# showlab/EgoVLP

Hardware: NVIDIA H100
Metric: clips/sec, 16-frame TimeSformer-B + DistilBERT + EgoNCE training step (higher is better)
Workload: dtype bf16

## Files before the change

### egovlp_b200/csrc/common.cuh

```cuda
#pragma once
#include <cuda.h>
#include <cuda_bf16.h>
#include <cuda_runtime.h>
#include <stdint.h>
#include <stdio.h>

#define EGOVLP_OK 0
#define EGOVLP_ERR_ARG (-1)
#define EGOVLP_ERR_CUDA (-2)
#define EGOVLP_ERR_UNSUPPORTED (-3)

namespace egovlp {

typedef __nv_bfloat16 bf16;

void set_last_error(const char* fmt, ...);

#define EGOVLP_CHECK_ARG(cond, ...)                                   \
  do {                                                                \
    if (!(cond)) {                                                    \
      ::egovlp::set_last_error(__VA_ARGS__);                          \
      return EGOVLP_ERR_ARG;                                          \
    }                                                                 \
  } while (0)
// ... 126 lines not shown
      "cp.async.bulk.tensor.2d.shared::cluster.global.mbarrier::complete_tx::bytes [%0], [%1, {%3, %4}], [%2];"
      ::"r"(dst), "l"(reinterpret_cast<uint64_t>(m)), "r"(bar), "r"(c0), "r"(c1)
      : "memory");
}
__device__ __forceinline__ void tma_load_3d(uint32_t dst, const CUtensorMap* m, uint32_t bar, int c0, int c1, int c2) {
  asm volatile(
      "cp.async.bulk.tensor.3d.shared::cluster.global.mbarrier::complete_tx::bytes [%0], [%1, {%3, %4, %5}], [%2];"
      ::"r"(dst), "l"(reinterpret_cast<uint64_t>(m)), "r"(bar), "r"(c0), "r"(c1), "r"(c2)
      : "memory");
}
__device__ __forceinline__ void tma_load_4d(uint32_t dst, const CUtensorMap* m, uint32_t bar, int c0, int c1, int c2,
                                            int c3) {
  asm volatile(
      "cp.async.bulk.tensor.4d.shared::cluster.global.mbarrier::complete_tx::bytes [%0], [%1, {%3, %4, %5, %6}], [%2];"
      ::"r"(dst), "l"(reinterpret_cast<uint64_t>(m)), "r"(bar), "r"(c0), "r"(c1), "r"(c2), "r"(c3)
      : "memory");
}
__device__ __forceinline__ void tma_load_5d(uint32_t dst, const CUtensorMap* m, uint32_t bar, int c0, int c1, int c2,
                                            int c3, int c4) {
  asm volatile(
      "cp.async.bulk.tensor.5d.shared::cluster.global.mbarrier::complete_tx::bytes [%0], [%1, {%3, %4, %5, %6, %7}], [%2];"
      ::"r"(dst), "l"(reinterpret_cast<uint64_t>(m)), "r"(bar), "r"(c0), "r"(c1), "r"(c2), "r"(c3), "r"(c4)
      : "memory");
}
__device__ __forceinline__ void tma_load_2d_multicast(uint32_t dst, const CUtensorMap* m, uint32_t bar, int c0, int c1,
                                                      uint16_t mask) {
  asm volatile(
      "cp.async.bulk.tensor.2d.shared::cluster.global.mbarrier::complete_tx::bytes.multicast::cluster"
      " [%0], [%1, {%3, %4}], [%2], %5;"
      ::"r"(dst), "l"(reinterpret_cast<uint64_t>(m)), "r"(bar), "r"(c0), "r"(c1), "h"(mask)
      : "memory");
}
__device__ __forceinline__ void fence_proxy_async_smem() {
  asm volatile("fence.proxy.async.shared::cta;" ::: "memory");
}
__device__ __forceinline__ void bulk_load_1d(uint32_t dst, const void* src, uint32_t bytes, uint32_t bar) {
  asm volatile("cp.async.bulk.shared::cluster.global.mbarrier::complete_tx::bytes [%0], [%1], %2, [%3];"
               ::"r"(dst), "l"(reinterpret_cast<uint64_t>(src)), "r"(bytes), "r"(bar)
               : "memory");
}
__device__ __forceinline__ void tma_store_2d(const CUtensorMap* m, uint32_t src, int c0, int c1) {
  asm volatile("cp.async.bulk.tensor.2d.global.shared::cta.bulk_group [%0, {%2, %3}], [%1];"
               ::"l"(reinterpret_cast<uint64_t>(m)), "r"(src), "r"(c0), "r"(c1)
               : "memory");
}
__device__ __forceinline__ void bulk_commit() { asm volatile("cp.async.bulk.commit_group;" ::: "memory"); }
template <int N>
__device__ __forceinline__ void bulk_wait_read() { asm volatile("cp.async.bulk.wait_group.read %0;" ::"n"(N) : "memory"); }
template <int N>
__device__ __forceinline__ void bulk_wait() { asm volatile("cp.async.bulk.wait_group %0;" ::"n"(N) : "memory"); }
__device__ __forceinline__ void named_bar_sync(int id, int count) {
  asm volatile("bar.sync %0, %1;" ::"r"(id), "r"(count) : "memory");
}

__device__ __forceinline__ uint32_t cluster_ctarank() {
  uint32_t r;
  asm volatile("mov.u32 %0, %%cluster_ctarank;" : "=r"(r));
  return r;
}
__device__ __forceinline__ void cluster_sync_all() {
  asm volatile("barrier.cluster.arrive.release.aligned;\n\tbarrier.cluster.wait.acquire.aligned;" ::: "memory");
}
__device__ __forceinline__ uint32_t mapa_shared(uint32_t addr, uint32_t cta_rank) {
  uint32_t r;
  asm volatile("mapa.shared::cluster.u32 %0, %1, %2;" : "=r"(r) : "r"(addr), "r"(cta_rank));
  return r;
}
__device__ __forceinline__ void mbar_arrive_cluster(uint32_t cluster_addr) {
  asm volatile("mbarrier.arrive.release.cluster.shared::cluster.b64 _, [%0];" ::"r"(cluster_addr) : "memory");
}

__device__ __forceinline__ void wgmma_fence() { asm volatile("wgmma.fence.sync.aligned;" ::: "memory"); }
__device__ __forceinline__ void wgmma_commit() { asm volatile("wgmma.commit_group.sync.aligned;" ::: "memory"); }
template <int N>
__device__ __forceinline__ void wgmma_wait() { asm volatile("wgmma.wait_group.sync.aligned %0;" ::"n"(N) : "memory"); }
template <int R>
__device__ __forceinline__ void wgmma_fence_regs(float (&d)[R]) {
#pragma unroll
  for (int i = 0; i < R; ++i) asm volatile("" : "+f"(d[i])::"memory");
}

__device__ __forceinline__ uint64_t make_smem_desc_sw128(uint32_t saddr, uint32_t lbo_bytes, uint32_t sbo_bytes) {
  uint64_t d = 0;
  d |= uint64_t((saddr >> 4) & 0x3FFF);
  d |= uint64_t((lbo_bytes >> 4) & 0x3FFF) << 16;
  d |= uint64_t((sbo_bytes >> 4) & 0x3FFF) << 32;
  d |= uint64_t(1) << 62;
  return d;
}

int make_tmap_2d_bf16(CUtensorMap* out, const void* base, uint64_t rows, uint64_t cols, uint64_t ld, uint32_t box_rows,
                      uint32_t box_cols);
int make_tmap_2d_f32(CUtensorMap* out, const void* base, uint64_t rows, uint64_t cols, uint64_t ld, uint32_t box_rows,
                     uint32_t box_cols);
int make_tmap_nd_bf16(CUtensorMap* out, const void* base, int rank, const uint64_t* dims, const uint64_t* strides,
                      const uint32_t* box, bool swizzle128);

}
```

### egovlp_b200/csrc/gemm_wgmma.cu

```cuda
#include <stdlib.h>

#include "common.cuh"
#include "egovlp_b200.h"

namespace egovlp {

namespace {

constexpr int BLOCK_M = 128;
constexpr int BLOCK_K = 64;
constexpr int WG_K = 16;
constexpr int A_STAGE_BYTES = BLOCK_M * BLOCK_K * 2;
constexpr int MN_ATOM_BYTES = BLOCK_K * 128;
constexpr int NUM_THREADS = 384;

struct EpiParams {
  const float* bias;
  const float* residual;
  const bf16* aux;
  void* out;
  bf16* out2;
  long long ldr, ldaux, ldo, ldo2;
  int out_mode;
  int act;
  float alpha;
  float col_scale;
  int col_scale_ncols;
  int res_row_mod;
  float* colsum;
  float* colsum_a;
};

constexpr int EPI_ROWS = 64;
constexpr int EPI_SUB_BYTES = EPI_ROWS * 128;
constexpr int EPI_BUFS = 2;
constexpr int EPI_BIAS_BYTES = 256 * 4;
constexpr int EPI_SMEM_BYTES = 2 * EPI_BUFS * EPI_SUB_BYTES + EPI_BIAS_BYTES;

template <int BLOCK_N>
struct Cfg {
  static constexpr int B_STAGE_BYTES = BLOCK_N * BLOCK_K * 2;
  static constexpr int STAGES = BLOCK_N == 256 ? 4 : 6;
  static constexpr int ACC = BLOCK_N / 2;
  static constexpr int RING_BYTES = STAGES * (A_STAGE_BYTES + B_STAGE_BYTES);
  static constexpr int SMEM_BYTES = RING_BYTES + 1024  + 256 ;
  static constexpr int SMEM_BYTES_STAGED = SMEM_BYTES + EPI_SMEM_BYTES;
  static_assert(SMEM_BYTES_STAGED <= 232448, "shared memory per block");
};

__device__ __forceinline__ void red_add_v4(float* p, float a, float b, float c, float d) {
  asm volatile("red.global.add.v4.f32 [%0], {%1, %2, %3, %4};" ::"l"(p), "f"(a), "f"(b), "f"(c), "f"(d) : "memory");
}
__device__ __forceinline__ void red_add_v2(float* p, float a, float b) {
  asm volatile("red.global.add.v2.f32 [%0], {%1, %2};" ::"l"(p), "f"(a), "f"(b) : "memory");
}

template <int TA, int TB>
__device__ __forceinline__ void wgmma_m64n256k16(float (&d)[128], uint64_t adesc, uint64_t bdesc, int scale_d) {
  asm volatile(
      "{\n\t.reg .pred p;\n\t"
      "setp.ne.b32 p, %130, 0;\n\t"
      "wgmma.mma_async.sync.aligned.m64n256k16.f32.bf16.bf16 "
      "{%0,%1,%2,%3,%4,%5,%6,%7,%8,%9,%10,%11,%12,%13,%14,%15,%16,%17,%18,%19,%20,%21,%22,%23,%24,%25,%26,%27,%28,%29,%30,%31,"
      "%32,%33,%34,%35,%36,%37,%38,%39,%40,%41,%42,%43,%44,%45,%46,%47,%48,%49,%50,%51,%52,%53,%54,%55,%56,%57,%58,%59,%60,%61,%62,%63,"
      "%64,%65,%66,%67,%68,%69,%70,%71,%72,%73,%74,%75,%76,%77,%78,%79,%80,%81,%82,%83,%84,%85,%86,%87,%88,%89,%90,%91,%92,%93,%94,%95,"
      "%96,%97,%98,%99,%100,%101,%102,%103,%104,%105,%106,%107,%108,%109,%110,%111,%112,%113,%114,%115,%116,%117,%118,%119,%120,%121,%122,%123,%124,%125,%126,%127}, "
      "%128, %129, p, 1, 1, %131, %132;\n\t}"
      : "+f"(d[0]), "+f"(d[1]), "+f"(d[2]), "+f"(d[3]), "+f"(d[4]), "+f"(d[5]), "+f"(d[6]), "+f"(d[7]),
        "+f"(d[8]), "+f"(d[9]), "+f"(d[10]), "+f"(d[11]), "+f"(d[12]), "+f"(d[13]), "+f"(d[14]), "+f"(d[15]),
        "+f"(d[16]), "+f"(d[17]), "+f"(d[18]), "+f"(d[19]), "+f"(d[20]), "+f"(d[21]), "+f"(d[22]), "+f"(d[23]),
        "+f"(d[24]), "+f"(d[25]), "+f"(d[26]), "+f"(d[27]), "+f"(d[28]), "+f"(d[29]), "+f"(d[30]), "+f"(d[31]),
        "+f"(d[32]), "+f"(d[33]), "+f"(d[34]), "+f"(d[35]), "+f"(d[36]), "+f"(d[37]), "+f"(d[38]), "+f"(d[39]),
        "+f"(d[40]), "+f"(d[41]), "+f"(d[42]), "+f"(d[43]), "+f"(d[44]), "+f"(d[45]), "+f"(d[46]), "+f"(d[47]),
        "+f"(d[48]), "+f"(d[49]), "+f"(d[50]), "+f"(d[51]), "+f"(d[52]), "+f"(d[53]), "+f"(d[54]), "+f"(d[55]),
        "+f"(d[56]), "+f"(d[57]), "+f"(d[58]), "+f"(d[59]), "+f"(d[60]), "+f"(d[61]), "+f"(d[62]), "+f"(d[63]),
        "+f"(d[64]), "+f"(d[65]), "+f"(d[66]), "+f"(d[67]), "+f"(d[68]), "+f"(d[69]), "+f"(d[70]), "+f"(d[71]),
        "+f"(d[72]), "+f"(d[73]), "+f"(d[74]), "+f"(d[75]), "+f"(d[76]), "+f"(d[77]), "+f"(d[78]), "+f"(d[79]),
        "+f"(d[80]), "+f"(d[81]), "+f"(d[82]), "+f"(d[83]), "+f"(d[84]), "+f"(d[85]), "+f"(d[86]), "+f"(d[87]),
        "+f"(d[88]), "+f"(d[89]), "+f"(d[90]), "+f"(d[91]), "+f"(d[92]), "+f"(d[93]), "+f"(d[94]), "+f"(d[95]),
        "+f"(d[96]), "+f"(d[97]), "+f"(d[98]), "+f"(d[99]), "+f"(d[100]), "+f"(d[101]), "+f"(d[102]), "+f"(d[103]),
        "+f"(d[104]), "+f"(d[105]), "+f"(d[106]), "+f"(d[107]), "+f"(d[108]), "+f"(d[109]), "+f"(d[110]), "+f"(d[111]),
        "+f"(d[112]), "+f"(d[113]), "+f"(d[114]), "+f"(d[115]), "+f"(d[116]), "+f"(d[117]), "+f"(d[118]), "+f"(d[119]),
        "+f"(d[120]), "+f"(d[121]), "+f"(d[122]), "+f"(d[123]), "+f"(d[124]), "+f"(d[125]), "+f"(d[126]), "+f"(d[127])
      : "l"(adesc), "l"(bdesc), "r"(scale_d), "n"(TA), "n"(TB));
}
template <int TA, int TB>
__device__ __forceinline__ void wgmma_m64n128k16(float (&d)[64], uint64_t adesc, uint64_t bdesc, int scale_d) {
  asm volatile(
      "{\n\t.reg .pred p;\n\t"
// ... 35 lines not shown
  u = mul2(x, gc.k);
  float u0, u1, a0, a1, t0, t1, e0, e1, r0, r1;
  up2(u, u0, u1);
  asm("rcp.approx.ftz.f32 %0, %1;" : "=f"(t0) : "f"(fmaf(fabsf(u0), GELU_PT, 1.f)));
  asm("rcp.approx.ftz.f32 %0, %1;" : "=f"(t1) : "f"(fmaf(fabsf(u1), GELU_PT, 1.f)));
  up2(fma2(mul2(x, gc.nk), u, gc.l2c), a0, a1);
  asm("ex2.approx.ftz.f32 %0, %1;" : "=f"(e0) : "f"(a0));
  asm("ex2.approx.ftz.f32 %0, %1;" : "=f"(e1) : "f"(a1));
  const f32x2 t = pk2(t0, t1);
  e = pk2(e0, e1);
  f32x2 p = fma2(t, gc.b5, gc.b4);
  p = fma2(p, t, gc.b3);
  p = fma2(p, t, gc.b2);
  p = fma2(p, t, gc.b1);
  up2(fma2(mul2(p, t), e, gc.half), r0, r1);
  return add2(pk2(copysignf(r0, x0), copysignf(r1, x1)), gc.half);
}
__device__ __forceinline__ void gelu2(const GeluConsts& gc, float& x0, float& x1) {
  const f32x2 x = pk2(x0, x1);
  f32x2 u, e;
  up2(mul2(x, gelu_phi2(gc, x0, x1, x, u, e)), x0, x1);
}
__device__ __forceinline__ void gelu_and_grad2(const GeluConsts& gc, float x0, float x1, uint32_t& g_bf, uint32_t& d_bf) {
  const f32x2 x = pk2(x0, x1);
  f32x2 u, e;
  const f32x2 phi = gelu_phi2(gc, x0, x1, x, u, e);
  float g0, g1, d0, d1;
  up2(mul2(x, phi), g0, g1);
  up2(fma2(u, e, phi), d0, d1);
  g_bf = pack_bf16x2(g0, g1);
  d_bf = pack_bf16x2(d0, d1);
}
__device__ __forceinline__ float gelu_grad_fast(float x) {
  float t;
  asm("rcp.approx.ftz.f32 %0, %1;" : "=f"(t) : "f"(fmaf(fabsf(x), 0.3275911f * 0.70710678118654752f, 1.f)));
  const float e = exp2f(x * x * -0.72134752044448170f);
  float p = fmaf(t, 0.5f * 1.061405429f, 0.5f * -1.453152027f);
  p = fmaf(p, t, 0.5f * 1.421413741f);
  p = fmaf(p, t, 0.5f * -0.284496736f);
  p = fmaf(p, t, 0.5f * 0.254829592f);
  const float phi_cdf = 0.5f + copysignf(fmaf(-(p * t), e, 0.5f), x);
  return fmaf(x * 0.3989422804014327f, e, phi_cdf);
}

enum EpiMode {
  EPI_GENERIC = 0,
  EPI_BF16 = 1,
  EPI_ACT3 = 2,
  EPI_MUL_AUX = 3,
  EPI_RES_F32 = 4,
  EPI_ACT1 = 5,
};

template <int BLOCK_N, bool A_MN, bool B_MN, bool TWO, int MODE>
__global__ void __launch_bounds__(NUM_THREADS, 1)
gemm_bf16_wgmma_kernel(const __grid_constant__ CUtensorMap tmA, const __grid_constant__ CUtensorMap tmB,
                       const __grid_constant__ CUtensorMap tmOut, const __grid_constant__ CUtensorMap tmOut2,
                       const __grid_constant__ CUtensorMap tmIn, int M, int N, int K, int num_m_blocks,
                       int num_n_blocks, int kb_per_split, int num_splits, EpiParams ep) {
  static_assert(!(TWO && A_MN && B_MN), "the wgrad form (column sums of A) runs on single CTAs");
  using C = Cfg<BLOCK_N>;
  constexpr int TILE_M = TWO ? 2 * BLOCK_M : BLOCK_M;
  const uint32_t rank = TWO ? cluster_ctarank() : 0u;
  const int worker = TWO ? (int)(blockIdx.x >> 1) : (int)blockIdx.x;
  const int num_workers = TWO ? (int)(gridDim.x >> 1) : (int)gridDim.x;
  constexpr int STAGES = C::STAGES;
  constexpr bool STAGED = MODE != EPI_GENERIC;
  constexpr bool OUT_F32 = MODE == EPI_RES_F32;
  constexpr bool HAS_IN = MODE == EPI_RES_F32 || MODE == EPI_MUL_AUX;
  constexpr bool TWO_OUT = MODE == EPI_ACT3;
  constexpr int SUB_COLS = OUT_F32 ? 32 : 64;
  constexpr int NSUB = BLOCK_N / SUB_COLS;
  extern __shared__ uint8_t smem_raw[];
  const uint32_t smem_base = (smem_u32(smem_raw) + 1023u) & ~1023u;
  const uint32_t sA = smem_base;
  const uint32_t sB = smem_base + STAGES * A_STAGE_BYTES;
  const uint32_t sEpi = sB + STAGES * C::B_STAGE_BYTES;
  const uint32_t sBias = sEpi + 2 * EPI_BUFS * EPI_SUB_BYTES;
  const uint32_t bars = STAGED ? sBias + EPI_BIAS_BYTES : sEpi;
  const uint32_t full_bar = bars;
  const uint32_t empty_bar = bars + 8 * STAGES;
  const uint32_t epi_full = bars + 16 * STAGES;
  const uint32_t epi_empty = epi_full + 8 * 2 * EPI_BUFS;
  const uint32_t bias_full = epi_empty + 8 * 2 * EPI_BUFS;
  const uint32_t bias_empty = bias_full + 8;

  const int warp = threadIdx.x >> 5;
  const int lane = threadIdx.x & 31;
  const int num_tiles = num_m_blocks * num_n_blocks;
  const int num_units = num_tiles * num_splits;
  const int num_kb = (K + BLOCK_K - 1) / BLOCK_K;
  const bool sum_a = A_MN && B_MN && ep.colsum_a != nullptr;

  if (threadIdx.x == 0) {
    tma_prefetch_desc(&tmA);
    tma_prefetch_desc(&tmB);
    for (int s = 0; s < STAGES; ++s) {
      mbar_init(full_bar + 8 * s, 1);
      mbar_init(empty_bar + 8 * s, (TWO || sum_a) ? 4 : 2);
    }
    if (STAGED) {
      tma_prefetch_desc(&tmOut);
      if (TWO_OUT) tma_prefetch_desc(&tmOut2);
      if (HAS_IN) tma_prefetch_desc(&tmIn);
      for (int i = 0; i < 2 * EPI_BUFS; ++i) {
        mbar_init(epi_full + 8 * i, 1);
        mbar_init(epi_empty + 8 * i, 1);
      }
      mbar_init(bias_full, 1);
      mbar_init(bias_empty, 2);
    }
    fence_mbar_init();
  }
  if (STAGED && !ep.bias && threadIdx.x < BLOCK_N)
    asm volatile("st.shared.f32 [%0], %1;" ::"r"(sBias + 4 * threadIdx.x), "f"(0.f) : "memory");
  if (TWO) cluster_sync_all();
  else __syncthreads();

  if (warp < 4) {
    asm volatile("setmaxnreg.dec.sync.aligned.u32 40;");
    if (warp == 0) {
      if (lane == 0) {
        int stage = 0;
        uint32_t phase = 0;
        for (int unit = worker; unit < num_units; unit += num_workers) {
          const int split = unit / num_tiles, tile = unit - split * num_tiles;
          const int m_blk = tile / num_n_blocks, n_blk = tile - m_blk * num_n_blocks;
          const int kb0 = split * kb_per_split, kb1 = min(num_kb, kb0 + kb_per_split);
          const int m_row = m_blk * TILE_M + (int)rank * BLOCK_M, n_row = n_blk * BLOCK_N;
          for (int kb = kb0; kb < kb1; ++kb) {
            mbar_wait_nocall(empty_bar + 8 * stage, phase ^ 1);
            const uint32_t fb = full_bar + 8 * stage;
            mbar_expect_tx(fb, A_STAGE_BYTES + C::B_STAGE_BYTES);
            const uint32_t a_dst = sA + stage * A_STAGE_BYTES, b_dst = sB + stage * C::B_STAGE_BYTES;
            if (!A_MN) {
              tma_load_2d(a_dst, &tmA, fb, kb * BLOCK_K, m_row);
            } else {
#pragma unroll
              for (int i = 0; i < BLOCK_M / 64; ++i)
                tma_load_2d(a_dst + i * MN_ATOM_BYTES, &tmA, fb, m_row + i * 64, kb * BLOCK_K);
            }
            if (TWO) {
              if (!B_MN) {
                tma_load_2d_multicast(b_dst + rank * (BLOCK_N / 2) * 128, &tmB, fb, kb * BLOCK_K,
                                      n_row + (int)rank * (BLOCK_N / 2), 3);
              } else {
#pragma unroll
                for (int i = 0; i < BLOCK_N / 128; ++i) {
                  const int slab = (int)rank * (BLOCK_N / 128) + i;
                  tma_load_2d_multicast(b_dst + slab * MN_ATOM_BYTES, &tmB, fb, n_row + slab * 64, kb * BLOCK_K, 3);
                }
              }
            } else if (!B_MN) {
              tma_load_2d(b_dst, &tmB, fb, kb * BLOCK_K, n_row);
            } else {
#pragma unroll
              for (int i = 0; i < BLOCK_N / 64; ++i)
                tma_load_2d(b_dst + i * MN_ATOM_BYTES, &tmB, fb, n_row + i * 64, kb * BLOCK_K);
            }
            if (++stage == STAGES) { stage = 0; phase ^= 1; }
          }
        }
      }
    } else if ((warp == 2 || warp == 3) && sum_a) {
      const int slab = warp - 2, chunk = lane & 7, rsub = lane >> 3;
      int stage = 0;
      uint32_t phase = 0;
      for (int unit = worker; unit < num_units; unit += num_workers) {
        const int split = unit / num_tiles, tile = unit - split * num_tiles;
        const int m_blk = tile / num_n_blocks, n_blk = tile - m_blk * num_n_blocks;
        const int kb0 = split * kb_per_split, kb1 = min(num_kb, kb0 + kb_per_split);
        float acc[8];
#pragma unroll
        for (int j = 0; j < 8; ++j) acc[j] = 0.f;
        for (int kb = kb0; kb < kb1; ++kb) {
          mbar_wait_nocall(full_bar + 8 * stage, phase);
          if (kb % num_n_blocks == n_blk) {
            const uint32_t slab_base = sA + stage * A_STAGE_BYTES + slab * MN_ATOM_BYTES;
#pragma unroll 4
            for (int i = 0; i < 16; ++i) {
              const int r = rsub + 4 * i;
              uint32_t v0, v1, v2, v3;
              asm volatile("ld.shared.v4.u32 {%0, %1, %2, %3}, [%4];"
                           : "=r"(v0), "=r"(v1), "=r"(v2), "=r"(v3)
                           : "r"(slab_base + r * 128 + ((chunk ^ (r & 7)) << 4)));
              acc[0] += __uint_as_float(v0 << 16); acc[1] += __uint_as_float(v0 & 0xffff0000u);
              acc[2] += __uint_as_float(v1 << 16); acc[3] += __uint_as_float(v1 & 0xffff0000u);
              acc[4] += __uint_as_float(v2 << 16); acc[5] += __uint_as_float(v2 & 0xffff0000u);
              acc[6] += __uint_as_float(v3 << 16); acc[7] += __uint_as_float(v3 & 0xffff0000u);
            }
          }
          __syncwarp();
          if (lane == 0) mbar_arrive(empty_bar + 8 * stage);
          if (++stage == STAGES) { stage = 0; phase ^= 1; }
        }
#pragma unroll
        for (int j = 0; j < 8; ++j) {
          acc[j] += __shfl_xor_sync(0xffffffffu, acc[j], 8);
          acc[j] += __shfl_xor_sync(0xffffffffu, acc[j], 16);
        }
        const int col = m_blk * BLOCK_M + slab * 64 + chunk * 8;
        if (lane < 8 && col < M) {
          red_add_v4(ep.colsum_a + col, acc[0], acc[1], acc[2], acc[3]);
          red_add_v4(ep.colsum_a + col + 4, acc[4], acc[5], acc[6], acc[7]);
        }
      }
    } else if (STAGED && warp == 1) {
      if (lane == 0) {
        uint32_t it = 0, tc = 0;
        for (int unit = worker; unit < num_units; unit += num_workers, ++tc) {
          const int m_blk = unit / num_n_blocks, n_blk = unit - m_blk * num_n_blocks;
          const int m_row = m_blk * TILE_M + (int)rank * BLOCK_M, n0 = n_blk * BLOCK_N;
          mbar_wait_nocall(bias_empty, (tc & 1) ^ 1);
          if (ep.bias) {
            const uint32_t bytes = 4u * (uint32_t)min(BLOCK_N, N - n0);
            mbar_expect_tx(bias_full, bytes);
            bulk_load_1d(sBias, ep.bias + n0, bytes, bias_full);
          } else {
            mbar_arrive(bias_full);
          }
          if (HAS_IN) {
            for (int s = 0; s < NSUB; ++s, ++it) {
              const uint32_t b = it % EPI_BUFS, ph = (it / EPI_BUFS) & 1;
#pragma unroll
              for (int w = 0; w < 2; ++w) {
                const uint32_t slot = w * EPI_BUFS + b;
                mbar_wait_nocall(epi_empty + 8 * slot, ph ^ 1);
                mbar_expect_tx(epi_full + 8 * slot, EPI_SUB_BYTES);
                tma_load_2d(sEpi + slot * EPI_SUB_BYTES, &tmIn, epi_full + 8 * slot, n0 + s * SUB_COLS,
                            m_row + w * EPI_ROWS);
              }
            }
          }
        }
      }
    }
  } else {
    asm volatile("setmaxnreg.inc.sync.aligned.u32 232;");
    const int mw = (threadIdx.x >> 7) - 1;
    const bool leader = (threadIdx.x & 127) == 0;
    auto release = [&](int st) {
      const uint32_t bar = empty_bar + 8 * st;
      if (TWO) { mbar_arrive_cluster(mapa_shared(bar, 0)); mbar_arrive_cluster(mapa_shared(bar, 1)); }
      else mbar_arrive(bar);
    };
    const int wq = warp & 3;
    const GeluConsts gc;

    float acc[C::ACC];
    int stage = 0;
    uint32_t phase = 0;
    uint32_t it = 0, tc = 0;
    for (int unit = worker; unit < num_units; unit += num_workers, ++tc) {
      const int split = unit / num_tiles, tile = unit - split * num_tiles;
      const int m_blk = tile / num_n_blocks, n_blk = tile - m_blk * num_n_blocks;
      const int kb0 = split * kb_per_split, kb1 = min(num_kb, kb0 + kb_per_split);
      int prev_stage = -1;
      for (int kb = kb0; kb < kb1; ++kb) {
        mbar_wait_nocall(full_bar + 8 * stage, phase);
        const uint32_t a_src = sA + stage * A_STAGE_BYTES + mw * (64 * 128), b_src = sB + stage * C::B_STAGE_BYTES;
        wgmma_fence_regs(acc);
        wgmma_fence();
#pragma unroll
        for (int k = 0; k < BLOCK_K / WG_K; ++k) {
          const uint64_t adesc = A_MN ? make_smem_desc_sw128(a_src + k * (WG_K * 128), MN_ATOM_BYTES, 1024)
                                      : make_smem_desc_sw128(a_src + k * (WG_K * 2), 16, 1024);
          const uint64_t bdesc = B_MN ? make_smem_desc_sw128(b_src + k * (WG_K * 128), MN_ATOM_BYTES, 1024)
                                      : make_smem_desc_sw128(b_src + k * (WG_K * 2), 16, 1024);
          wgmma_tile<BLOCK_N, A_MN ? 1 : 0, B_MN ? 1 : 0>(acc, adesc, bdesc, (kb > kb0 || k > 0) ? 1 : 0);
        }
        wgmma_commit();
        wgmma_fence_regs(acc);
        wgmma_wait<1>();
        wgmma_fence_regs(acc);
        if (prev_stage >= 0 && leader) release(prev_stage);
        prev_stage = stage;
        if (++stage == STAGES) { stage = 0; phase ^= 1; }
      }
      wgmma_wait<0>();
      wgmma_fence_regs(acc);
      if (leader) release(prev_stage);

      if constexpr (STAGED) {
        const int m_row = m_blk * TILE_M + (int)rank * BLOCK_M + mw * EPI_ROWS, n0 = n_blk * BLOCK_N;
        const int c2 = 2 * (lane & 3);
        mbar_wait_nocall(bias_full, tc & 1);
#pragma unroll
        for (int s = 0; s < NSUB; ++s, ++it) {
          const uint32_t b = it % EPI_BUFS, ph = (it / EPI_BUFS) & 1;
          if (TWO_OUT) named_bar_sync(1 + mw, 128);
          const uint32_t buf = sEpi + (mw * EPI_BUFS + (TWO_OUT ? 0u : b)) * EPI_SUB_BYTES;
          if (HAS_IN) mbar_wait_nocall(epi_full + 8 * (mw * EPI_BUFS + b), ph);
#pragma unroll
          for (int jj = 0; jj < SUB_COLS / 8; ++jj) {
            const int j = s * (SUB_COLS / 8) + jj;
            float2 bq;
            asm volatile("ld.shared.v2.f32 {%0, %1}, [%2];" : "=f"(bq.x), "=f"(bq.y) : "r"(sBias + 4 * (8 * j + c2)));
#pragma unroll
            for (int h = 0; h < 2; ++h) {
              const int r = wq * 16 + (lane >> 2) + 8 * h;
              const uint32_t off = OUT_F32 ? r * 128 + (((2 * jj + ((lane & 3) >> 1)) ^ (r & 7)) << 4) + 8 * (lane & 1)
                                           : r * 128 + ((jj ^ (r & 7)) << 4) + 4 * (lane & 3);
              float v0 = __fmaf_rn(acc[4 * j + 2 * h], ep.alpha, bq.x);
              float v1 = __fmaf_rn(acc[4 * j + 2 * h + 1], ep.alpha, bq.y);
              if (MODE == EPI_BF16 && n0 + 8 * j + c2 < ep.col_scale_ncols) {
                v0 = __fmul_rn(v0, ep.col_scale); v1 = __fmul_rn(v1, ep.col_scale);
              }
              if (MODE == EPI_ACT3) {
                uint32_t g, d;
                gelu_and_grad2(gc, v0, v1, g, d);
                asm volatile("st.shared.u32 [%0], %1;" ::"r"(buf + off), "r"(g) : "memory");
                asm volatile("st.shared.u32 [%0], %1;" ::"r"(buf + EPI_SUB_BYTES + off), "r"(d) : "memory");
              } else if (MODE == EPI_RES_F32) {
                float r0, r1;
                asm volatile("ld.shared.v2.f32 {%0, %1}, [%2];" : "=f"(r0), "=f"(r1) : "r"(buf + off) : "memory");
                v0 += r0; v1 += r1;
                asm volatile("st.shared.v2.f32 [%0], {%1, %2};" ::"r"(buf + off), "f"(v0), "f"(v1) : "memory");
              } else {
                if (MODE == EPI_ACT1) gelu2(gc, v0, v1);
                if (MODE == EPI_MUL_AUX) {
                  uint32_t a;
                  asm volatile("ld.shared.u32 %0, [%1];" : "=r"(a) : "r"(buf + off) : "memory");
                  const float2 af = unpack_bf16x2(a);
                  v0 *= af.x; v1 *= af.y;
                }
                asm volatile("st.shared.u32 [%0], %1;" ::"r"(buf + off), "r"(pack_bf16x2(v0, v1)) : "memory");
              }
            }
          }
          fence_proxy_async_smem();
          named_bar_sync(1 + mw, 128);
          if (leader) {
            tma_store_2d(&tmOut, buf, n0 + s * SUB_COLS, m_row);
            if (TWO_OUT) tma_store_2d(&tmOut2, buf + EPI_SUB_BYTES, n0 + s * SUB_COLS, m_row);
            bulk_commit();
            bulk_wait_read<0>();
            if (HAS_IN) mbar_arrive(epi_empty + 8 * (mw * EPI_BUFS + b));
          }
        }
        if (leader) mbar_arrive(bias_empty);
      } else {
      const int row_lo = m_blk * TILE_M + (int)rank * BLOCK_M + mw * 64 + wq * 16 + (lane >> 2);
      const int col_base = n_blk * BLOCK_N + 2 * (lane & 3);
#pragma unroll
      for (int j = 0; j < BLOCK_N / 8; ++j) {
        const int col = col_base + 8 * j;
        if (n_blk * BLOCK_N + 8 * j >= N) break;
        float2 bq = make_float2(0.f, 0.f);
        if (ep.bias) bq = __ldg(reinterpret_cast<const float2*>(ep.bias + col));
        float cs0 = 0.f, cs1 = 0.f;
#pragma unroll
        for (int h = 0; h < 2; ++h) {
          const int row = row_lo + 8 * h;
          const bool rv = row < M;
          float v0 = __fmaf_rn(acc[4 * j + 2 * h], ep.alpha, bq.x);
          float v1 = __fmaf_rn(acc[4 * j + 2 * h + 1], ep.alpha, bq.y);
          if (col < ep.col_scale_ncols) { v0 = __fmul_rn(v0, ep.col_scale); v1 = __fmul_rn(v1, ep.col_scale); }
          if (ep.act == 3) {
            uint32_t g, d;
            gelu_and_grad2(gc, v0, v1, g, d);
            if (rv) {
              *reinterpret_cast<uint32_t*>(reinterpret_cast<bf16*>(ep.out) + (long long)row * ep.ldo + col) = g;
              if (ep.out2) *reinterpret_cast<uint32_t*>(ep.out2 + (long long)row * ep.ldo2 + col) = d;
            }
            continue;
          }
          if (ep.out2 && rv)
            *reinterpret_cast<uint32_t*>(ep.out2 + (long long)row * ep.ldo2 + col) = pack_bf16x2(v0, v1);
          if (ep.act == 1) gelu2(gc, v0, v1);
          const int grow = rv ? row : M - 1;
          if (ep.act == 2 || ep.act == 4) {
            const float2 a = unpack_bf16x2(__ldg(reinterpret_cast<const unsigned int*>(ep.aux + (long long)grow * ep.ldaux + col)));
            if (ep.act == 2) { v0 *= gelu_grad_fast(a.x); v1 *= gelu_grad_fast(a.y); }
            else { v0 *= a.x; v1 *= a.y; }
          }
          if (ep.residual) {
            const int rrow = ep.res_row_mod ? grow % ep.res_row_mod : grow;
            const float2 r = __ldg(reinterpret_cast<const float2*>(ep.residual + (long long)rrow * ep.ldr + col));
            v0 += r.x; v1 += r.y;
          }
          if (!rv) continue;
          cs0 += v0; cs1 += v1;
          if (ep.out_mode == 0) {
            *reinterpret_cast<uint32_t*>(reinterpret_cast<bf16*>(ep.out) + (long long)row * ep.ldo + col) = pack_bf16x2(v0, v1);
          } else if (ep.out_mode == 1) {
            *reinterpret_cast<float2*>(reinterpret_cast<float*>(ep.out) + (long long)row * ep.ldo + col) = make_float2(v0, v1);
          } else {
            red_add_v2(reinterpret_cast<float*>(ep.out) + (long long)row * ep.ldo + col, v0, v1);
          }
        }
        if (ep.colsum) {
#pragma unroll
          for (int o = 4; o < 32; o <<= 1) {
            cs0 += __shfl_xor_sync(0xffffffffu, cs0, o);
            cs1 += __shfl_xor_sync(0xffffffffu, cs1, o);
          }
          if (lane < 4) red_add_v2(ep.colsum + col, cs0, cs1);
        }
      }
      }
    }
    if (STAGED && leader) bulk_wait<0>();
  }
  if (TWO) cluster_sync_all();
}

template <int BLOCK_N, bool A_MN, bool B_MN, bool TWO, int MODE = EPI_GENERIC>
int launch(const void* A, long long lda, const void* B, long long ldb, int M, int N, int K, int splits,
           const EpiParams& ep, cudaStream_t stream) {
  using C = Cfg<BLOCK_N>;
  CUtensorMap tmA, tmB;
  int rc;
  if (!A_MN) rc = make_tmap_2d_bf16(&tmA, A, M, K, lda, BLOCK_M, BLOCK_K);
  else       rc = make_tmap_2d_bf16(&tmA, A, K, M, lda, BLOCK_K, 64);
  if (rc) return rc;
  if (!B_MN) rc = make_tmap_2d_bf16(&tmB, B, N, K, ldb, TWO ? BLOCK_N / 2 : BLOCK_N, BLOCK_K);
  else       rc = make_tmap_2d_bf16(&tmB, B, K, N, ldb, BLOCK_K, 64);
  if (rc) return rc;
  constexpr bool STAGED = MODE != EPI_GENERIC;
  CUtensorMap tmOut = {}, tmOut2 = {}, tmIn = {};
  if (MODE == EPI_RES_F32) {
    rc = make_tmap_2d_f32(&tmOut, ep.out, M, N, ep.ldo, EPI_ROWS, 32);
    if (!rc) rc = make_tmap_2d_f32(&tmIn, ep.residual, M, N, ep.ldr, EPI_ROWS, 32);
  } else if (STAGED) {
    rc = make_tmap_2d_bf16(&tmOut, ep.out, M, N, ep.ldo, EPI_ROWS, 64);
    if (!rc && MODE == EPI_ACT3) rc = make_tmap_2d_bf16(&tmOut2, ep.out2, M, N, ep.ldo2, EPI_ROWS, 64);
    if (!rc && MODE == EPI_MUL_AUX) rc = make_tmap_2d_bf16(&tmIn, ep.aux, M, N, ep.ldaux, EPI_ROWS, 64);
  }
  if (rc) return rc;
  constexpr int SMEM_BYTES = STAGED ? C::SMEM_BYTES_STAGED : C::SMEM_BYTES;
  constexpr int TILE_M = TWO ? 2 * BLOCK_M : BLOCK_M;
  const int num_m_blocks = (M + TILE_M - 1) / TILE_M, num_n_blocks = (N + BLOCK_N - 1) / BLOCK_N;
  const int num_kb = (K + BLOCK_K - 1) / BLOCK_K;
  splits = max(1, min(splits, num_kb));
  const int kb_per_split = (num_kb + splits - 1) / splits;
  splits = (num_kb + kb_per_split - 1) / kb_per_split;
  const int units = num_m_blocks * num_n_blocks * splits;
  auto kern = gemm_bf16_wgmma_kernel<BLOCK_N, A_MN, B_MN, TWO, MODE>;
  static bool attr_set = false;
  if (!attr_set) {
    EGOVLP_CHECK_CUDA(cudaFuncSetAttribute(kern, cudaFuncAttributeMaxDynamicSharedMemorySize, SMEM_BYTES));
    attr_set = true;
  }
  cudaLaunchConfig_t cfg = {};
  cudaLaunchAttribute attr[1];
  cfg.blockDim = dim3(NUM_THREADS);
  cfg.dynamicSmemBytes = SMEM_BYTES;
  cfg.stream = stream;
  if (TWO) {
    attr[0].id = cudaLaunchAttributeClusterDimension;
    attr[0].val.clusterDim.x = 2;
    attr[0].val.clusterDim.y = 1;
    attr[0].val.clusterDim.z = 1;
    cfg.attrs = attr;
    cfg.numAttrs = 1;
  }
  static int resident = 0;
  if (!resident) {
    if (TWO) {
      cfg.gridDim = dim3(num_sms() & ~1);
      EGOVLP_CHECK_CUDA(cudaOccupancyMaxActiveClusters(&resident, kern, &cfg));
      if (resident < 1) resident = 1;
    } else {
      resident = num_sms();
    }
  }
  const int workers = min(units, resident);
  cfg.gridDim = dim3(TWO ? 2 * workers : workers);
  EGOVLP_CHECK_CUDA(cudaLaunchKernelEx(&cfg, kern, tmA, tmB, tmOut, tmOut2, tmIn, M, N, K, num_m_blocks, num_n_blocks,
                                       kb_per_split, splits, ep));
  return EGOVLP_OK;
}

template <int BLOCK_N, bool TWO, int MODE = EPI_GENERIC>
int dispatch_major(int a_mn, int b_mn, const void* A, long long lda, const void* B, long long ldb, int M, int N, int K,
                   int splits, const EpiParams& ep, cudaStream_t stream) {
  if (!a_mn && !b_mn) return launch<BLOCK_N, false, false, TWO, MODE>(A, lda, B, ldb, M, N, K, splits, ep, stream);
  if (!a_mn && b_mn) return launch<BLOCK_N, false, true, TWO, MODE>(A, lda, B, ldb, M, N, K, splits, ep, stream);
  if (a_mn && b_mn) return launch<BLOCK_N, true, true, false, EPI_GENERIC>(A, lda, B, ldb, M, N, K, splits, ep, stream);
  return launch<BLOCK_N, true, false, false, EPI_GENERIC>(A, lda, B, ldb, M, N, K, splits, ep, stream);
}

inline bool tma_ok(const void* p, long long ld_bytes) {
  return (reinterpret_cast<uintptr_t>(p) & 15) == 0 && ld_bytes % 16 == 0;
}

inline int epi_mode(const EpiParams& ep) {
  const char* g = getenv("EGOVLP_GEMM_GENERIC_EPI");
  if (g && g[0] == '1') return EPI_GENERIC;
  if (ep.colsum || ep.res_row_mod) return EPI_GENERIC;
  if (ep.bias && (reinterpret_cast<uintptr_t>(ep.bias) & 15) != 0) return EPI_GENERIC;
  const bool no_scale = ep.col_scale_ncols == 0;
  const bool out16 = tma_ok(ep.out, ep.ldo * 2);
  if (ep.act == 0 && ep.out_mode == 0 && !ep.residual && !ep.out2 && out16) return EPI_BF16;
  if (ep.act == 3 && ep.out_mode == 0 && !ep.residual && ep.out2 && no_scale && out16 && tma_ok(ep.out2, ep.ldo2 * 2))
    return EPI_ACT3;
  if (ep.act == 4 && ep.out_mode == 0 && !ep.residual && !ep.out2 && no_scale && out16 && tma_ok(ep.aux, ep.ldaux * 2))
    return EPI_MUL_AUX;
  if (ep.act == 0 && ep.out_mode == 1 && ep.residual && !ep.out2 && no_scale && tma_ok(ep.out, ep.ldo * 4) &&
      tma_ok(ep.residual, ep.ldr * 4))
    return EPI_RES_F32;
  if (ep.act == 1 && ep.out_mode == 0 && !ep.residual && !ep.out2 && no_scale && out16) return EPI_ACT1;
  return EPI_GENERIC;
}

inline bool use_pairs() {
  const char* e = getenv("EGOVLP_GEMM_PAIR");
  return e && e[0] == '1';
}

template <int BLOCK_N, bool TWO>
int dispatch_mode(int a_mn, int b_mn, const void* A, long long lda, const void* B, long long ldb, int M, int N, int K,
                  int splits, const EpiParams& ep, cudaStream_t stream) {
  if (!a_mn) {
    switch (epi_mode(ep)) {
      case EPI_BF16: return dispatch_major<BLOCK_N, TWO, EPI_BF16>(a_mn, b_mn, A, lda, B, ldb, M, N, K, splits, ep, stream);
      case EPI_ACT3: return dispatch_major<BLOCK_N, TWO, EPI_ACT3>(a_mn, b_mn, A, lda, B, ldb, M, N, K, splits, ep, stream);
      case EPI_MUL_AUX: return dispatch_major<BLOCK_N, TWO, EPI_MUL_AUX>(a_mn, b_mn, A, lda, B, ldb, M, N, K, splits, ep, stream);
      case EPI_RES_F32: return dispatch_major<BLOCK_N, TWO, EPI_RES_F32>(a_mn, b_mn, A, lda, B, ldb, M, N, K, splits, ep, stream);
      case EPI_ACT1: return dispatch_major<BLOCK_N, TWO, EPI_ACT1>(a_mn, b_mn, A, lda, B, ldb, M, N, K, splits, ep, stream);
      default: break;
    }
  }
  return dispatch_major<BLOCK_N, TWO>(a_mn, b_mn, A, lda, B, ldb, M, N, K, splits, ep, stream);
}

}

}

using namespace egovlp;

extern "C" int egovlp_gemm_bf16(const void* A, int a_mn_major, long long lda, const void* B, int b_mn_major,
                                long long ldb, int M, int N, int K, const egovlp_gemm_epilogue* e, int split_k,
                                void* stream) {
  EGOVLP_CHECK_ARG(A && B && e && e->out, "gemm: null pointer");
  EGOVLP_CHECK_ARG(M > 0 && N > 0 && K > 0, "gemm: bad shape M=%d N=%d K=%d", M, N, K);
  EGOVLP_CHECK_ARG(N % 32 == 0, "gemm: N=%d must be a multiple of 32", N);
  EGOVLP_CHECK_ARG(lda % 8 == 0 && ldb % 8 == 0, "gemm: leading dimensions must be multiples of 8 (16B TMA strides)");
  EGOVLP_CHECK_ARG((reinterpret_cast<uintptr_t>(A) & 15) == 0 && (reinterpret_cast<uintptr_t>(B) & 15) == 0,
                   "gemm: operands must be 16B aligned");
  EGOVLP_CHECK_ARG(e->out_mode >= 0 && e->out_mode <= 2 && e->act >= 0 && e->act <= 4, "gemm: bad epilogue mode");
  EGOVLP_CHECK_ARG(split_k <= 1 || e->out_mode == 2, "gemm: split_k > 1 needs out_mode=2 (fp32 atomic accumulate)");
  EGOVLP_CHECK_ARG((e->act != 2 && e->act != 4) || e->aux, "gemm: act=2/4 needs aux");
  EGOVLP_CHECK_ARG(e->ldo % 8 == 0, "gemm: ldo must be a multiple of 8");
  EpiParams ep;
  ep.bias = e->bias; ep.residual = e->residual; ep.aux = reinterpret_cast<const bf16*>(e->aux);
  ep.out = e->out; ep.out2 = reinterpret_cast<bf16*>(e->out2);
  ep.ldr = e->ldr; ep.ldaux = e->ldaux; ep.ldo = e->ldo; ep.ldo2 = e->ldo2;
  ep.out_mode = e->out_mode; ep.act = e->act; ep.alpha = e->alpha;
  ep.col_scale = e->col_scale; ep.col_scale_ncols = e->col_scale_ncols; ep.res_row_mod = e->res_row_mod;
  ep.colsum = e->colsum;
  ep.colsum_a = e->colsum_a;
  EGOVLP_CHECK_ARG(!e->colsum_a || (a_mn_major && b_mn_major && N % 256 == 0 && M % 8 == 0 &&
                                    (reinterpret_cast<uintptr_t>(e->colsum_a) & 15) == 0),
                   "gemm: colsum_a needs the MN/MN (wgrad) form with N % 256 == 0, M % 8 == 0 and a 16B-aligned vector");
  cudaStream_t st = reinterpret_cast<cudaStream_t>(stream);
  if (N % 256 == 0 && !a_mn_major && use_pairs())
    return dispatch_mode<256, true>(a_mn_major, b_mn_major, A, lda, B, ldb, M, N, K, split_k, ep, st);
  if (N % 256 == 0) return dispatch_mode<256, false>(a_mn_major, b_mn_major, A, lda, B, ldb, M, N, K, split_k, ep, st);
  return dispatch_mode<128, false>(a_mn_major, b_mn_major, A, lda, B, ldb, M, N, K, split_k, ep, st);
}
```

Baseline: 134.3.

## Add ping-pong consumer schedule for GEMMs with aux-multiply epilogues

Measured after the change: 134.1, median of 6. About the same (-0.2%).

```diff
diff --git a/egovlp_b200/csrc/common.cuh b/egovlp_b200/csrc/common.cuh
--- a/egovlp_b200/csrc/common.cuh
+++ b/egovlp_b200/csrc/common.cuh
@@ -202,6 +202,9 @@
 __device__ __forceinline__ void named_bar_sync(int id, int count) {
   asm volatile("bar.sync %0, %1;" ::"r"(id), "r"(count) : "memory");
 }
+__device__ __forceinline__ void named_bar_arrive(int id, int count) {
+  asm volatile("bar.arrive %0, %1;" ::"r"(id), "r"(count) : "memory");
+}
 
 __device__ __forceinline__ uint32_t cluster_ctarank() {
   uint32_t r;
diff --git a/egovlp_b200/csrc/gemm_wgmma.cu b/egovlp_b200/csrc/gemm_wgmma.cu
--- a/egovlp_b200/csrc/gemm_wgmma.cu
+++ b/egovlp_b200/csrc/gemm_wgmma.cu
@@ -35,6 +35,7 @@
 constexpr int EPI_SUB_BYTES = EPI_ROWS * 128;
 constexpr int EPI_BUFS = 2;
 constexpr int EPI_BIAS_BYTES = 256 * 4;
+constexpr int ORDER_BAR = 3;
 constexpr int EPI_SMEM_BYTES = 2 * EPI_BUFS * EPI_SUB_BYTES + EPI_BIAS_BYTES;
 
 template <int BLOCK_N>
@@ -176,14 +177,16 @@
   EPI_ACT1 = 5,
 };
 
-template <int BLOCK_N, bool A_MN, bool B_MN, bool TWO, int MODE>
+template <int BLOCK_N, bool A_MN, bool B_MN, bool TWO, int MODE, bool PP>
 __global__ void __launch_bounds__(NUM_THREADS, 1)
 gemm_bf16_wgmma_kernel(const __grid_constant__ CUtensorMap tmA, const __grid_constant__ CUtensorMap tmB,
                        const __grid_constant__ CUtensorMap tmOut, const __grid_constant__ CUtensorMap tmOut2,
                        const __grid_constant__ CUtensorMap tmIn, int M, int N, int K, int num_m_blocks,
                        int num_n_blocks, int kb_per_split, int num_splits, EpiParams ep) {
   static_assert(!(TWO && A_MN && B_MN), "the wgrad form (column sums of A) runs on single CTAs");
+  static_assert(!PP || (BLOCK_N == 128 && !A_MN && !TWO), "ping-pong: 128 x 128 tiles, K-major A, single CTAs");
   using C = Cfg<BLOCK_N>;
+  constexpr int RH = PP ? 2 : 1;
   constexpr int TILE_M = TWO ? 2 * BLOCK_M : BLOCK_M;
   const uint32_t rank = TWO ? cluster_ctarank() : 0u;
   const int worker = TWO ? (int)(blockIdx.x >> 1) : (int)blockIdx.x;
@@ -194,7 +197,8 @@
   constexpr bool HAS_IN = MODE == EPI_RES_F32 || MODE == EPI_MUL_AUX;
   constexpr bool TWO_OUT = MODE == EPI_ACT3;
   constexpr int SUB_COLS = OUT_F32 ? 32 : 64;
-  constexpr int NSUB = BLOCK_N / SUB_COLS;
+  constexpr int NSUB_N = BLOCK_N / SUB_COLS;
+  constexpr int NSUB = RH * NSUB_N;
   extern __shared__ uint8_t smem_raw[];
   const uint32_t smem_base = (smem_u32(smem_raw) + 1023u) & ~1023u;
   const uint32_t sA = smem_base;
@@ -207,7 +211,8 @@
   const uint32_t epi_full = bars + 16 * STAGES;
   const uint32_t epi_empty = epi_full + 8 * 2 * EPI_BUFS;
   const uint32_t bias_full = epi_empty + 8 * 2 * EPI_BUFS;
-  const uint32_t bias_empty = bias_full + 8;
+  const uint32_t bias_empty = bias_full + 8 * RH;
+  static_assert(16 * STAGES + 32 * EPI_BUFS + 16 * RH <= 256, "barrier area");
 
   const int warp = threadIdx.x >> 5;
   const int lane = threadIdx.x & 31;
@@ -221,7 +226,7 @@
     tma_prefetch_desc(&tmB);
     for (int s = 0; s < STAGES; ++s) {
       mbar_init(full_bar + 8 * s, 1);
-      mbar_init(empty_bar + 8 * s, (TWO || sum_a) ? 4 : 2);
+      mbar_init(empty_bar + 8 * s, PP ? 1 : (TWO || sum_a) ? 4 : 2);
     }
     if (STAGED) {
       tma_prefetch_desc(&tmOut);
@@ -231,12 +236,14 @@
         mbar_init(epi_full + 8 * i, 1);
         mbar_init(epi_empty + 8 * i, 1);
       }
-      mbar_init(bias_full, 1);
-      mbar_init(bias_empty, 2);
+      for (int i = 0; i < RH; ++i) {
+        mbar_init(bias_full + 8 * i, 1);
+        mbar_init(bias_empty + 8 * i, PP ? 1 : 2);
+      }
     }
     fence_mbar_init();
   }
-  if (STAGED && !ep.bias && threadIdx.x < BLOCK_N)
+  if (STAGED && !ep.bias && threadIdx.x < EPI_BIAS_BYTES / 4)
     asm volatile("st.shared.f32 [%0], %1;" ::"r"(sBias + 4 * threadIdx.x), "f"(0.f) : "memory");
   if (TWO) cluster_sync_all();
   else __syncthreads();
@@ -331,28 +338,31 @@
       }
     } else if (STAGED && warp == 1) {
       if (lane == 0) {
-        uint32_t it = 0, tc = 0;
+        uint32_t tc = 0;
         for (int unit = worker; unit < num_units; unit += num_workers, ++tc) {
           const int m_blk = unit / num_n_blocks, n_blk = unit - m_blk * num_n_blocks;
           const int m_row = m_blk * TILE_M + (int)rank * BLOCK_M, n0 = n_blk * BLOCK_N;
-          mbar_wait_nocall(bias_empty, (tc & 1) ^ 1);
+          const uint32_t w = PP ? (tc & 1) : 0u, own = PP ? (tc >> 1) : tc;
+          const uint32_t bfull = bias_full + 8 * w;
+          mbar_wait_nocall(bias_empty + 8 * w, (own & 1) ^ 1);
           if (ep.bias) {
             const uint32_t bytes = 4u * (uint32_t)min(BLOCK_N, N - n0);
-            mbar_expect_tx(bias_full, bytes);
-            bulk_load_1d(sBias, ep.bias + n0, bytes, bias_full);
+            mbar_expect_tx(bfull, bytes);
+            bulk_load_1d(sBias + w * (BLOCK_N * 4), ep.bias + n0, bytes, bfull);
           } else {
-            mbar_arrive(bias_full);
+            mbar_arrive(bfull);
           }
           if (HAS_IN) {
-            for (int s = 0; s < NSUB; ++s, ++it) {
-              const uint32_t b = it % EPI_BUFS, ph = (it / EPI_BUFS) & 1;
-#pragma unroll
-              for (int w = 0; w < 2; ++w) {
-                const uint32_t slot = w * EPI_BUFS + b;
+            for (int s = 0; s < NSUB; ++s) {
+              const uint32_t it = own * NSUB + s, b = it % EPI_BUFS, ph = (it / EPI_BUFS) & 1;
+              const int col = n0 + (s % NSUB_N) * SUB_COLS;
+#pragma unroll
+              for (int v = 0; v < (PP ? 1 : 2); ++v) {
+                const uint32_t slot = (PP ? w : (uint32_t)v) * EPI_BUFS + b;
+                const int row = m_row + (PP ? s / NSUB_N : v) * EPI_ROWS;
                 mbar_wait_nocall(epi_empty + 8 * slot, ph ^ 1);
                 mbar_expect_tx(epi_full + 8 * slot, EPI_SUB_BYTES);
-                tma_load_2d(sEpi + slot * EPI_SUB_BYTES, &tmIn, epi_full + 8 * slot, n0 + s * SUB_COLS,
-                            m_row + w * EPI_ROWS);
+                tma_load_2d(sEpi + slot * EPI_SUB_BYTES, &tmIn, epi_full + 8 * slot, col, row);
               }
             }
           }
@@ -371,62 +381,81 @@
     const int wq = warp & 3;
     const GeluConsts gc;
 
-    float acc[C::ACC];
+    float acc[RH][C::ACC];
+    auto fence_acc = [&]() {
+#pragma unroll
+      for (int rh = 0; rh < RH; ++rh) wgmma_fence_regs(acc[rh]);
+    };
     int stage = 0;
     uint32_t phase = 0;
-    uint32_t it = 0, tc = 0;
+    uint32_t tc = 0;
     for (int unit = worker; unit < num_units; unit += num_workers, ++tc) {
       const int split = unit / num_tiles, tile = unit - split * num_tiles;
       const int m_blk = tile / num_n_blocks, n_blk = tile - m_blk * num_n_blocks;
       const int kb0 = split * kb_per_split, kb1 = min(num_kb, kb0 + kb_per_split);
+      if (PP && (int)(tc & 1) != mw) {
+        stage += kb1 - kb0;
+        while (stage >= STAGES) { stage -= STAGES; phase ^= 1; }
+        continue;
+      }
+      const uint32_t own = PP ? tc >> 1 : tc;
+      if (PP && tc > 0) named_bar_sync(ORDER_BAR + mw, 256);
       int prev_stage = -1;
       for (int kb = kb0; kb < kb1; ++kb) {
         mbar_wait_nocall(full_bar + 8 * stage, phase);
-        const uint32_t a_src = sA + stage * A_STAGE_BYTES + mw * (64 * 128), b_src = sB + stage * C::B_STAGE_BYTES;
-        wgmma_fence_regs(acc);
+        const uint32_t a_src = sA + stage * A_STAGE_BYTES + (PP ? 0 : mw * (64 * 128));
+        const uint32_t b_src = sB + stage * C::B_STAGE_BYTES;
+        fence_acc();
         wgmma_fence();
 #pragma unroll
         for (int k = 0; k < BLOCK_K / WG_K; ++k) {
-          const uint64_t adesc = A_MN ? make_smem_desc_sw128(a_src + k * (WG_K * 128), MN_ATOM_BYTES, 1024)
-                                      : make_smem_desc_sw128(a_src + k * (WG_K * 2), 16, 1024);
           const uint64_t bdesc = B_MN ? make_smem_desc_sw128(b_src + k * (WG_K * 128), MN_ATOM_BYTES, 1024)
                                       : make_smem_desc_sw128(b_src + k * (WG_K * 2), 16, 1024);
-          wgmma_tile<BLOCK_N, A_MN ? 1 : 0, B_MN ? 1 : 0>(acc, adesc, bdesc, (kb > kb0 || k > 0) ? 1 : 0);
+#pragma unroll
+          for (int rh = 0; rh < RH; ++rh) {
+            const uint32_t a_rows = a_src + rh * (64 * 128);
+            const uint64_t adesc = A_MN ? make_smem_desc_sw128(a_rows + k * (WG_K * 128), MN_ATOM_BYTES, 1024)
+                                        : make_smem_desc_sw128(a_rows + k * (WG_K * 2), 16, 1024);
+            wgmma_tile<BLOCK_N, A_MN ? 1 : 0, B_MN ? 1 : 0>(acc[rh], adesc, bdesc, (kb > kb0 || k > 0) ? 1 : 0);
+          }
         }
         wgmma_commit();
-        wgmma_fence_regs(acc);
+        fence_acc();
         wgmma_wait<1>();
-        wgmma_fence_regs(acc);
+        fence_acc();
         if (prev_stage >= 0 && leader) release(prev_stage);
         prev_stage = stage;
         if (++stage == STAGES) { stage = 0; phase ^= 1; }
       }
+      if (PP && unit + num_workers < num_units) named_bar_arrive(ORDER_BAR + (mw ^ 1), 256);
       wgmma_wait<0>();
-      wgmma_fence_regs(acc);
+      fence_acc();
       if (leader) release(prev_stage);
 
       if constexpr (STAGED) {
-        const int m_row = m_blk * TILE_M + (int)rank * BLOCK_M + mw * EPI_ROWS, n0 = n_blk * BLOCK_N;
+        const int m_row = m_blk * TILE_M + (int)rank * BLOCK_M + (PP ? 0 : mw * EPI_ROWS), n0 = n_blk * BLOCK_N;
         const int c2 = 2 * (lane & 3);
-        mbar_wait_nocall(bias_full, tc & 1);
-#pragma unroll
-        for (int s = 0; s < NSUB; ++s, ++it) {
-          const uint32_t b = it % EPI_BUFS, ph = (it / EPI_BUFS) & 1;
+        const uint32_t bias_row = sBias + (PP ? mw * (BLOCK_N * 4) : 0);
+        mbar_wait_nocall(bias_full + (PP ? 8 * mw : 0), own & 1);
+#pragma unroll
+        for (int s = 0; s < NSUB; ++s) {
+          const int rh = s / NSUB_N, cs = s % NSUB_N;
+          const uint32_t it = own * NSUB + s, b = it % EPI_BUFS, ph = (it / EPI_BUFS) & 1;
           if (TWO_OUT) named_bar_sync(1 + mw, 128);
           const uint32_t buf = sEpi + (mw * EPI_BUFS + (TWO_OUT ? 0u : b)) * EPI_SUB_BYTES;
           if (HAS_IN) mbar_wait_nocall(epi_full + 8 * (mw * EPI_BUFS + b), ph);
 #pragma unroll
           for (int jj = 0; jj < SUB_COLS / 8; ++jj) {
-            const int j = s * (SUB_COLS / 8) + jj;
+            const int j = cs * (SUB_COLS / 8) + jj;
             float2 bq;
-            asm volatile("ld.shared.v2.f32 {%0, %1}, [%2];" : "=f"(bq.x), "=f"(bq.y) : "r"(sBias + 4 * (8 * j + c2)));
+            asm volatile("ld.shared.v2.f32 {%0, %1}, [%2];" : "=f"(bq.x), "=f"(bq.y) : "r"(bias_row + 4 * (8 * j + c2)));
 #pragma unroll
             for (int h = 0; h < 2; ++h) {
               const int r = wq * 16 + (lane >> 2) + 8 * h;
               const uint32_t off = OUT_F32 ? r * 128 + (((2 * jj + ((lane & 3) >> 1)) ^ (r & 7)) << 4) + 8 * (lane & 1)
                                            : r * 128 + ((jj ^ (r & 7)) << 4) + 4 * (lane & 3);
-              float v0 = __fmaf_rn(acc[4 * j + 2 * h], ep.alpha, bq.x);
-              float v1 = __fmaf_rn(acc[4 * j + 2 * h + 1], ep.alpha, bq.y);
+              float v0 = __fmaf_rn(acc[rh][4 * j + 2 * h], ep.alpha, bq.x);
+              float v1 = __fmaf_rn(acc[rh][4 * j + 2 * h + 1], ep.alpha, bq.y);
               if (MODE == EPI_BF16 && n0 + 8 * j + c2 < ep.col_scale_ncols) {
                 v0 = __fmul_rn(v0, ep.col_scale); v1 = __fmul_rn(v1, ep.col_scale);
               }
@@ -455,16 +484,18 @@
           fence_proxy_async_smem();
           named_bar_sync(1 + mw, 128);
           if (leader) {
-            tma_store_2d(&tmOut, buf, n0 + s * SUB_COLS, m_row);
-            if (TWO_OUT) tma_store_2d(&tmOut2, buf + EPI_SUB_BYTES, n0 + s * SUB_COLS, m_row);
+            tma_store_2d(&tmOut, buf, n0 + cs * SUB_COLS, m_row + rh * EPI_ROWS);
+            if (TWO_OUT) tma_store_2d(&tmOut2, buf + EPI_SUB_BYTES, n0 + cs * SUB_COLS, m_row + rh * EPI_ROWS);
             bulk_commit();
             bulk_wait_read<0>();
             if (HAS_IN) mbar_arrive(epi_empty + 8 * (mw * EPI_BUFS + b));
           }
         }
-        if (leader) mbar_arrive(bias_empty);
+        if (leader) mbar_arrive(bias_empty + (PP ? 8 * mw : 0));
       } else {
-      const int row_lo = m_blk * TILE_M + (int)rank * BLOCK_M + mw * 64 + wq * 16 + (lane >> 2);
+#pragma unroll
+      for (int rh = 0; rh < RH; ++rh) {
+      const int row_lo = m_blk * TILE_M + (int)rank * BLOCK_M + (PP ? rh : mw) * 64 + wq * 16 + (lane >> 2);
       const int col_base = n_blk * BLOCK_N + 2 * (lane & 3);
 #pragma unroll
       for (int j = 0; j < BLOCK_N / 8; ++j) {
@@ -477,8 +508,8 @@
         for (int h = 0; h < 2; ++h) {
           const int row = row_lo + 8 * h;
           const bool rv = row < M;
-          float v0 = __fmaf_rn(acc[4 * j + 2 * h], ep.alpha, bq.x);
-          float v1 = __fmaf_rn(acc[4 * j + 2 * h + 1], ep.alpha, bq.y);
+          float v0 = __fmaf_rn(acc[rh][4 * j + 2 * h], ep.alpha, bq.x);
+          float v1 = __fmaf_rn(acc[rh][4 * j + 2 * h + 1], ep.alpha, bq.y);
           if (col < ep.col_scale_ncols) { v0 = __fmul_rn(v0, ep.col_scale); v1 = __fmul_rn(v1, ep.col_scale); }
           if (ep.act == 3) {
             uint32_t g, d;
@@ -523,13 +554,14 @@
         }
       }
       }
+      }
     }
     if (STAGED && leader) bulk_wait<0>();
   }
   if (TWO) cluster_sync_all();
 }
 
-template <int BLOCK_N, bool A_MN, bool B_MN, bool TWO, int MODE = EPI_GENERIC>
+template <int BLOCK_N, bool A_MN, bool B_MN, bool TWO, int MODE = EPI_GENERIC, bool PP = false>
 int launch(const void* A, long long lda, const void* B, long long ldb, int M, int N, int K, int splits,
            const EpiParams& ep, cudaStream_t stream) {
   using C = Cfg<BLOCK_N>;
@@ -560,7 +592,7 @@
   const int kb_per_split = (num_kb + splits - 1) / splits;
   splits = (num_kb + kb_per_split - 1) / kb_per_split;
   const int units = num_m_blocks * num_n_blocks * splits;
-  auto kern = gemm_bf16_wgmma_kernel<BLOCK_N, A_MN, B_MN, TWO, MODE>;
+  auto kern = gemm_bf16_wgmma_kernel<BLOCK_N, A_MN, B_MN, TWO, MODE, PP>;
   static bool attr_set = false;
   if (!attr_set) {
     EGOVLP_CHECK_CUDA(cudaFuncSetAttribute(kern, cudaFuncAttributeMaxDynamicSharedMemorySize, SMEM_BYTES));
@@ -596,11 +628,11 @@
   return EGOVLP_OK;
 }
 
-template <int BLOCK_N, bool TWO, int MODE = EPI_GENERIC>
+template <int BLOCK_N, bool TWO, int MODE = EPI_GENERIC, bool PP = false>
 int dispatch_major(int a_mn, int b_mn, const void* A, long long lda, const void* B, long long ldb, int M, int N, int K,
                    int splits, const EpiParams& ep, cudaStream_t stream) {
-  if (!a_mn && !b_mn) return launch<BLOCK_N, false, false, TWO, MODE>(A, lda, B, ldb, M, N, K, splits, ep, stream);
-  if (!a_mn && b_mn) return launch<BLOCK_N, false, true, TWO, MODE>(A, lda, B, ldb, M, N, K, splits, ep, stream);
+  if (!a_mn && !b_mn) return launch<BLOCK_N, false, false, TWO, MODE, PP>(A, lda, B, ldb, M, N, K, splits, ep, stream);
+  if (!a_mn && b_mn) return launch<BLOCK_N, false, true, TWO, MODE, PP>(A, lda, B, ldb, M, N, K, splits, ep, stream);
   if (a_mn && b_mn) return launch<BLOCK_N, true, true, false, EPI_GENERIC>(A, lda, B, ldb, M, N, K, splits, ep, stream);
   return launch<BLOCK_N, true, false, false, EPI_GENERIC>(A, lda, B, ldb, M, N, K, splits, ep, stream);
 }
@@ -647,6 +679,16 @@
     }
   }
   return dispatch_major<BLOCK_N, TWO>(a_mn, b_mn, A, lda, B, ldb, M, N, K, splits, ep, stream);
+}
+
+inline bool use_pingpong(int a_mn, int N, const EpiParams& ep) {
+  return !a_mn && N % 128 == 0 && (ep.act == 2 || ep.act == 4);
+}
+int dispatch_pingpong(int b_mn, const void* A, long long lda, const void* B, long long ldb, int M, int N, int K,
+                      int splits, const EpiParams& ep, cudaStream_t stream) {
+  if (epi_mode(ep) == EPI_MUL_AUX)
+    return dispatch_major<128, false, EPI_MUL_AUX, true>(0, b_mn, A, lda, B, ldb, M, N, K, splits, ep, stream);
+  return dispatch_major<128, false, EPI_GENERIC, true>(0, b_mn, A, lda, B, ldb, M, N, K, splits, ep, stream);
 }
 
 }
@@ -682,6 +724,8 @@
   cudaStream_t st = reinterpret_cast<cudaStream_t>(stream);
   if (N % 256 == 0 && !a_mn_major && use_pairs())
     return dispatch_mode<256, true>(a_mn_major, b_mn_major, A, lda, B, ldb, M, N, K, split_k, ep, st);
+  if (use_pingpong(a_mn_major, N, ep))
+    return dispatch_pingpong(b_mn_major, A, lda, B, ldb, M, N, K, split_k, ep, st);
   if (N % 256 == 0) return dispatch_mode<256, false>(a_mn_major, b_mn_major, A, lda, B, ldb, M, N, K, split_k, ep, st);
   return dispatch_mode<128, false>(a_mn_major, b_mn_major, A, lda, B, ldb, M, N, K, split_k, ep, st);
 }
```
